# airframesio/aero-cli

Measured on AMD Instinct MI355X. Metric: Msamples/s demod+Viterbi, 10500bps OQPSK, 1/2/4/8 GPU; ACARS frames bit-exact vs ref, higher is better.
Workload: dtype f64

## Files before the change

### aero-cli_amd/aero_engine.py

```python
import ctypes
import os

import numpy as np

HERE = os.path.dirname(os.path.abspath(__file__))
LIB_PATH = os.path.join(HERE, 'libaero_engine.so')

AERO_OK = 0
AERO_E_INVALID = -1
AERO_E_NOMEM = -2
AERO_E_HIP = -3
AERO_E_NOGPU = -4
AERO_E_FULL = -5
AERO_E_RATE = -6
AERO_E_DEVICE = -7

F_TRACE_PT = 0x1
F_TRACE_BLOCKS = 0x2
F_TIMING = 0x4
F_TRACE_SOFT = 0x8
F_TRACE_HOPS = 0x10
F_TRACE_FRAMES = 0x20
F_DCD_TICK = 0x40
F_DCD_TICK_BURST = 0x80
F_DCD_TICK_CONT = 0x100
F_TRACE_ALL = F_TRACE_PT | F_TRACE_BLOCKS | F_TRACE_SOFT | F_TRACE_HOPS | F_TRACE_FRAMES

MATH_FN = {'hypot': 0, 'atan2': 1, 'tanh': 2, 'sin': 3, 'cos': 4, 'log10': 5, 'sqrt': 6, 'fmod360': 7,
           'div': 8, 'div_c48000': 9, 'div_c360': 10, 'div_n': 11, 'div_c192000': 13, 'hypot_nr': 14, 'atan2_bf': 15,
           'tanh_bf': 16, 'sin_bf': 17, 'cos_bf': 18,
           'div_cw_wt': 19, 'set_phase_ptr': 20, 'log10_ge1': 21}
VIT_VARIANT = {'wave': 0, 'regs': 1, 'regs2-self': 2, 'regs2-pair': 3, 'block4992': 4, 'block384': 5, 'block576': 6,
               'csoft': 7}
FFT_KIND = {'dit': 0, 'chain': 1}
VIT_BLOCK = {'block4992': 4992, 'block384': 384, 'block576': 576, 'csoft': 5460}


class EngineCfg(ctypes.Structure):
    _fields_ = [('device', ctypes.c_int), ('max_channels', ctypes.c_int), ('flags', ctypes.c_int)]


class ChannelCfg(ctypes.Structure):
    _fields_ = [('bitrate', ctypes.c_int), ('burst', ctypes.c_int), ('fs', ctypes.c_uint32),
                ('disable_reassembly', ctypes.c_int)]


class AcarsItem(ctypes.Structure):
    _fields_ = [('aesid', ctypes.c_uint32),
                ('gesid', ctypes.c_uint8), ('qno', ctypes.c_uint8), ('refno', ctypes.c_uint8),
                ('seqno', ctypes.c_uint8),
                ('mode', ctypes.c_uint8), ('tak', ctypes.c_uint8), ('bi', ctypes.c_uint8),
                ('nonacars', ctypes.c_uint8),
                ('downlink', ctypes.c_uint8), ('valid', ctypes.c_uint8), ('hastext', ctypes.c_uint8),
                ('moretocome', ctypes.c_uint8),
                ('fragment', ctypes.c_uint8), ('label_len', ctypes.c_uint8), ('reg_len', ctypes.c_uint8),
                ('pad0', ctypes.c_uint8),
                ('label', ctypes.c_char * 4), ('reg', ctypes.c_char * 16),
                ('msg_len', ctypes.c_uint32), ('msg', ctypes.c_char * 3584)]


class ChanCfg(ctypes.Structure):
    _fields_ = [('device', ctypes.c_int), ('sample_rate', ctypes.c_int), ('center_frequency', ctypes.c_int),
                ('mix_offset', ctypes.c_int), ('correct_dc_bias', ctypes.c_int), ('max_blocks', ctypes.c_int),
                ('flags', ctypes.c_int)]


class ChanMain(ctypes.Structure):
    _fields_ = [('frequency', ctypes.c_int), ('out_rate', ctypes.c_int), ('compress_scale', ctypes.c_int),
                ('publish', ctypes.c_int)]


class ChanVfo(ctypes.Structure):
    _fields_ = [('frequency', ctypes.c_int), ('data_rate', ctypes.c_int), ('out_rate', ctypes.c_int),
                ('filter_bandwidth', ctypes.c_int), ('gain', ctypes.c_float), ('skip', ctypes.c_int)]


CHAN_F_HOST_OUT = 0x1


class ChannelEvents(ctypes.Structure):
    _fields_ = [('dcd_edges', ctypes.c_int64), ('hunter_steps', ctypes.c_int64), ('hunter_fc', ctypes.c_double * 8)]


_SIGS = {
    'aero_engine_create': (ctypes.c_int, [ctypes.POINTER(EngineCfg), ctypes.POINTER(ctypes.c_void_p)]),
    'aero_engine_destroy': (None, [ctypes.c_void_p]),
    'aero_channel_open': (ctypes.c_int, [ctypes.c_void_p, ctypes.POINTER(ChannelCfg), ctypes.POINTER(ctypes.c_int)]),
    'aero_channel_close': (ctypes.c_int, [ctypes.c_void_p, ctypes.c_int]),
    'aero_engine_reserve': (ctypes.c_int, [ctypes.c_void_p, ctypes.POINTER(ChannelCfg), ctypes.c_int]),
    'aero_channel_export': (ctypes.c_int, [ctypes.c_void_p, ctypes.POINTER(ctypes.c_int), ctypes.c_int,
                                           ctypes.c_void_p, ctypes.c_size_t, ctypes.POINTER(ctypes.c_size_t)]),
    'aero_channel_import': (ctypes.c_int, [ctypes.c_void_p, ctypes.c_void_p, ctypes.c_size_t,
                                           ctypes.POINTER(ctypes.c_int), ctypes.c_int,
                                           ctypes.POINTER(ctypes.c_int)]),
    'aero_push_pcm': (ctypes.c_int, [ctypes.c_void_p, ctypes.c_int, ctypes.c_void_p, ctypes.c_size_t,
                                     ctypes.c_uint32]),
    'aero_push_pcm_batch': (ctypes.c_int, [ctypes.c_void_p, ctypes.c_void_p, ctypes.c_size_t, ctypes.c_size_t,
                                           ctypes.c_int, ctypes.c_int]),
    'aero_push_pcm_dev': (ctypes.c_int, [ctypes.c_void_p, ctypes.c_int, ctypes.c_void_p, ctypes.c_size_t,
                                         ctypes.c_uint32]),
    'aero_run': (ctypes.c_int, [ctypes.c_void_p]),
    'aero_flush': (ctypes.c_int, [ctypes.c_void_p]),
    'aero_pop_softbits': (ctypes.c_int, [ctypes.c_void_p, ctypes.c_int, ctypes.c_void_p, ctypes.c_size_t,
                                         ctypes.POINTER(ctypes.c_size_t)]),
    'aero_pop_items': (ctypes.c_int, [ctypes.c_void_p, ctypes.c_int, ctypes.POINTER(AcarsItem), ctypes.c_size_t,
                                      ctypes.POINTER(ctypes.c_size_t)]),
    'aero_pop_items_all': (ctypes.c_int, [ctypes.c_void_p, ctypes.POINTER(AcarsItem), ctypes.POINTER(ctypes.c_int),
                                          ctypes.c_size_t, ctypes.POINTER(ctypes.c_size_t)]),
    'aero_pop_hops': (ctypes.c_int, [ctypes.c_void_p, ctypes.c_int, ctypes.c_void_p, ctypes.c_size_t,
                                     ctypes.POINTER(ctypes.c_size_t)]),
    'aero_trace_select': (ctypes.c_int, [ctypes.c_void_p, ctypes.POINTER(ctypes.c_int), ctypes.c_int]),
    'aero_pop_pt': (ctypes.c_int, [ctypes.c_void_p, ctypes.c_int, ctypes.c_void_p, ctypes.c_size_t,
                                   ctypes.POINTER(ctypes.c_size_t)]),
    'aero_pop_blocks': (ctypes.c_int, [ctypes.c_void_p, ctypes.c_int, ctypes.c_void_p, ctypes.c_size_t,
                                       ctypes.POINTER(ctypes.c_size_t)]),
    'aero_pop_frames': (ctypes.c_int, [ctypes.c_void_p, ctypes.c_int, ctypes.c_void_p, ctypes.c_size_t,
                                       ctypes.POINTER(ctypes.c_size_t)]),
    'aero_pop_rt_tests': (ctypes.c_int, [ctypes.c_void_p, ctypes.c_int, ctypes.c_void_p, ctypes.c_size_t,
                                         ctypes.POINTER(ctypes.c_size_t)]),
    'aero_pop_c_units': (ctypes.c_int, [ctypes.c_void_p, ctypes.c_int, ctypes.c_void_p, ctypes.c_size_t,
                                        ctypes.POINTER(ctypes.c_size_t)]),
    'aero_pop_voice': (ctypes.c_int, [ctypes.c_void_p, ctypes.c_int, ctypes.c_void_p, ctypes.c_size_t,
                                      ctypes.POINTER(ctypes.c_size_t)]),
    'aero_pop_rt_packets': (ctypes.c_int, [ctypes.c_void_p, ctypes.c_int, ctypes.c_void_p, ctypes.c_size_t,
                                           ctypes.POINTER(ctypes.c_size_t)]),
    'aero_timing': (ctypes.c_int, [ctypes.c_void_p, ctypes.c_char_p, ctypes.POINTER(ctypes.c_double),
                                   ctypes.POINTER(ctypes.c_long)]),
    'aero_timing_reset': (None, [ctypes.c_void_p]),
    'aero_samples_processed': (ctypes.c_uint64, [ctypes.c_void_p]),
    'aero_stat': (ctypes.c_int, [ctypes.c_void_p, ctypes.c_char_p, ctypes.POINTER(ctypes.c_uint64)]),
    'aero_channel_stat': (ctypes.c_int, [ctypes.c_void_p, ctypes.c_int, ctypes.c_char_p,
                                         ctypes.POINTER(ctypes.c_int64)]),
    'aero_channel_get_events': (ctypes.c_int, [ctypes.c_void_p, ctypes.c_int, ctypes.POINTER(ChannelEvents)]),
    'aero_sync': (ctypes.c_int, [ctypes.c_void_p]),
    'aero_device_math': (ctypes.c_int, [ctypes.c_void_p, ctypes.c_int, ctypes.c_void_p, ctypes.c_void_p,
                                        ctypes.c_void_p, ctypes.c_size_t]),
    'aero_device_viterbi': (ctypes.c_int, [ctypes.c_void_p, ctypes.c_int, ctypes.c_void_p, ctypes.c_size_t,
                                           ctypes.c_size_t, ctypes.c_void_p, ctypes.c_void_p]),
    'aero_device_fft': (ctypes.c_int, [ctypes.c_void_p] + [ctypes.c_int] * 6 + [ctypes.c_void_p, ctypes.c_size_t,
                                                                                 ctypes.c_void_p]),
    'aero_channel_coarse_y': (ctypes.c_int, [ctypes.c_void_p, ctypes.c_int, ctypes.c_void_p, ctypes.c_size_t,
                                             ctypes.POINTER(ctypes.c_size_t), ctypes.POINTER(ctypes.c_int)]),
    'aero_strerror': (ctypes.c_char_p, [ctypes.c_int]),
    'aero_chan_create': (ctypes.c_int, [ctypes.POINTER(ChanCfg), ctypes.POINTER(ChanMain), ctypes.c_int,
                                        ctypes.POINTER(ChanVfo), ctypes.c_int, ctypes.POINTER(ctypes.c_void_p)]),
    'aero_chan_destroy': (None, [ctypes.c_void_p]),
    'aero_chan_block_len': (ctypes.c_int, [ctypes.c_void_p, ctypes.POINTER(ctypes.c_int)]),
    'aero_chan_vfo_info': (ctypes.c_int, [ctypes.c_void_p, ctypes.c_int, ctypes.POINTER(ctypes.c_int)]),
    'aero_chan_main_info': (ctypes.c_int, [ctypes.c_void_p, ctypes.c_int, ctypes.POINTER(ctypes.c_int)]),
    'aero_chan_push': (ctypes.c_int, [ctypes.c_void_p, ctypes.c_void_p, ctypes.c_size_t, ctypes.c_int]),
    'aero_chan_run': (ctypes.c_int, [ctypes.c_void_p]),
    'aero_chan_sync': (ctypes.c_int, [ctypes.c_void_p]),
    'aero_chan_vfo_output': (ctypes.c_int, [ctypes.c_void_p, ctypes.c_int, ctypes.POINTER(ctypes.c_void_p),
                                            ctypes.POINTER(ctypes.c_size_t)]),
    'aero_chan_pop_audio': (ctypes.c_int, [ctypes.c_void_p, ctypes.c_int, ctypes.c_void_p, ctypes.c_size_t,
                                           ctypes.POINTER(ctypes.c_size_t)]),
    'aero_chan_pop_iq': (ctypes.c_int, [ctypes.c_void_p, ctypes.c_int, ctypes.c_void_p, ctypes.c_size_t,
                                        ctypes.POINTER(ctypes.c_size_t)]),
    'aero_chan_feed': (ctypes.c_int, [ctypes.c_void_p, ctypes.c_void_p, ctypes.POINTER(ctypes.c_int)]),
    'aero_chan_vfo_open': (ctypes.c_int, [ctypes.c_void_p, ctypes.POINTER(ChanVfo), ctypes.POINTER(ctypes.c_int)]),
    'aero_chan_vfo_close': (ctypes.c_int, [ctypes.c_void_p, ctypes.c_int]),
    'aero_chan_vfo_skip': (ctypes.c_int, [ctypes.c_void_p, ctypes.c_int, ctypes.c_int]),
    'aero_chan_reserve': (ctypes.c_int, [ctypes.c_void_p, ctypes.POINTER(ChanVfo), ctypes.c_int]),
    'aero_chan_vfo_count': (ctypes.c_int, [ctypes.c_void_p, ctypes.POINTER(ctypes.c_int)]),
    'aero_chan_vfo_settle': (ctypes.c_int, [ctypes.c_void_p, ctypes.c_int, ctypes.POINTER(ctypes.c_size_t)]),
    'aero_chan_stat': (ctypes.c_int, [ctypes.c_void_p, ctypes.c_char_p, ctypes.POINTER(ctypes.c_uint64)]),
}

_lib = None


def _torch_hip_runtime():
    import importlib.util
    spec = importlib.util.find_spec('torch')
    if spec is None or not spec.origin:
        return []
    tlib = os.path.join(os.path.dirname(spec.origin), 'lib')
    return [p for p in (os.path.join(tlib, 'libhsa-runtime64.so'), os.path.join(tlib, 'libamdhip64.so'))
            if os.path.exists(p)]


def load_library(path=None):
    global _lib
    if _lib is not None:
        return _lib
    path = path or os.environ.get('AERO_ENGINE_SO') or LIB_PATH
    if not os.path.exists(path):
        raise RuntimeError('libaero_engine.so not built (%s); run aero-cli_amd/build.py' % path)
    for rt in _torch_hip_runtime():
        ctypes.CDLL(rt, mode=ctypes.RTLD_GLOBAL)
    lib = ctypes.CDLL(path)
    for name, (res, args) in _SIGS.items():
        try:
# ... 247 lines not shown
        self.lib.aero_timing_reset(self.h)

    def stat(self, name):
        v = ctypes.c_uint64()
        _check(self.lib.aero_stat(self.h, name.encode(), ctypes.byref(v)), 'aero_stat')
        return int(v.value)

    def channel_stat(self, ch, name):
        v = ctypes.c_int64()
        _check(self.lib.aero_channel_stat(self.h, ch, name.encode(), ctypes.byref(v)), 'aero_channel_stat')
        return int(v.value)

    def channel_events(self, ch):
        ev = ChannelEvents()
        _check(self.lib.aero_channel_get_events(self.h, ch, ctypes.byref(ev)), 'aero_channel_get_events')
        n = int(ev.hunter_steps)
        fcs = [ev.hunter_fc[(k - 1) & 7] for k in range(max(1, n - 7), n + 1)]
        return int(ev.dcd_edges), n, fcs

    def samples_processed(self):
        return int(self.lib.aero_samples_processed(self.h))

    def device_math(self, fn, x, y=None):
        x = np.ascontiguousarray(x, dtype=np.float64)
        y = np.zeros_like(x) if y is None else np.ascontiguousarray(y, dtype=np.float64)
        out = np.empty_like(x)
        _check(self.lib.aero_device_math(self.h, MATH_FN[fn], x.ctypes.data, y.ctypes.data, out.ctypes.data,
                                         x.size), 'aero_device_math')
        return out

    def device_viterbi(self, variant, rows, nsoft=None):
        rows = np.ascontiguousarray(rows, dtype=np.uint8)
        assert rows.ndim == 2
        src = variant in VIT_BLOCK
        nsoft = rows.shape[1] if nsoft is None else int(nsoft)
        bits = np.zeros((rows.shape[0], nsoft // 2), dtype=np.uint8)
        ov = np.zeros((rows.shape[0], 62), dtype=np.uint8)
        _check(self.lib.aero_device_viterbi(self.h, VIT_VARIANT[variant], rows.ctypes.data, rows.shape[0], nsoft,
                                            bits.ctypes.data, ov.ctypes.data if src else None),
               'aero_device_viterbi')
        return (bits, ov) if src else bits

    def device_fft(self, kind, records, inverse=False, depth=0, start=1, stop=0):
        records = np.ascontiguousarray(records, dtype=np.complex128)
        assert records.ndim == 2
        n = records.shape[1]
        log2n = n.bit_length() - 1 if n > 0 and n & (n - 1) == 0 else 0
        out = np.empty_like(records)
        _check(self.lib.aero_device_fft(self.h, FFT_KIND.get(kind, -1), log2n, int(inverse), int(depth), int(start),
                                        int(stop), records.ctypes.data, records.shape[0], out.ctypes.data),
               'aero_device_fft')
        return out

    def channel_coarse_y(self, ch):
        y = np.empty(16384, dtype=np.float64)
        n, first = ctypes.c_size_t(), ctypes.c_int()
        _check(self.lib.aero_channel_coarse_y(self.h, ch, y.ctypes.data, y.size, ctypes.byref(n), ctypes.byref(first)),
               'aero_channel_coarse_y')
        return int(first.value), y[:n.value].copy()


def vfo_out_rate(data_rate, out_rate=0):
    if out_rate or not data_rate:
        return out_rate
    return {600: 12000, 1200: 24000}.get(int(data_rate), 48000)


def vfo_bitrate(data_rate):
    return int(data_rate) if int(data_rate) in (600, 1200) else 10500


def parse_sdr_ini(text):
    sections, cur = {}, 'General'
    for raw in text.splitlines():
        line = raw.strip()
        if not line or line[0] in ';#':
            continue
        if line.startswith('[') and line.endswith(']'):
            cur = line[1:-1]
            continue
        if '=' in line:
            k, v = line.split('=', 1)
            sections.setdefault(cur, {})[k.strip()] = v.strip()

    def to_int(v):
        try:
            return int(v)
        except (TypeError, ValueError):
            return 0

    def to_float(v):
        try:
            return float(v)
        except (TypeError, ValueError):
            return 0.0

    def array(name):
        sec = sections.get(name, {})
        out = []
        for i in range(1, to_int(sec.get('size')) + 1):
            pre = '%d\\' % i
            out.append({k[len(pre):]: v for k, v in sec.items() if k.startswith(pre)})
        return out

    g = sections.get('General', {})
    general = dict(sample_rate=to_int(g.get('sample_rate')), center_frequency=to_int(g.get('center_frequency')),
# ... 142 lines not shown
```

### aero-cli_amd/build.py

```python
import argparse
import concurrent.futures as cf
import os
import shutil
import subprocess
import sys

HERE = os.path.dirname(os.path.abspath(__file__))
ROOT = os.path.dirname(HERE)
CSRC = os.path.join(HERE, 'csrc')
BUILD = os.path.join(HERE, 'build')
ENGINE_SO = os.path.join(HERE, 'libaero_engine.so')
SYNTH_SO = os.path.join(ROOT, 'tools', 'libaero_synth.so')
ORACLE_DIR = os.path.join(ROOT, 'oracle')

ARCH = os.environ.get('AERO_OFFLOAD_ARCH', 'gfx950')
HIPCC = os.environ.get('HIPCC', shutil.which('hipcc') or '/opt/rocm/bin/hipcc')
FP = ['-ffp-contract=off', '-fno-fast-math']
HIP_FLAGS = ['-O3', '-std=c++17', '-fPIC', '--offload-arch=' + ARCH] + FP
CXX_FLAGS = ['-O2', '-std=c++17', '-fPIC', '-Wall'] + FP

HIP_SRCS = ['demod_oqpsk.hip', 'demod_msk.hip', 'coarse.hip', 'aerol.hip', 'engine.hip', 'chan.hip', 'burst.hip', 'burst_msk.hip',
            'burst_engine.hip', 'cchan.hip', 'slot_reset.hip', 'slot_copy.hip', 'viterbi_probe.hip',
            'fft_probe.hip']
CXX_SRCS = ['tables_host.cpp', 'acars_host.cpp', 'chan_blob.cpp']
FILE_FLAGS = {'burst.hip': ['-mllvm', '-disable-machine-licm'],
              'burst_msk.hip': ['-mllvm', '-disable-machine-licm'],
              'demod_oqpsk.hip': ['-mllvm', '--amdgpu-sched-strategy=max-memory-clause', '-mllvm',
                                  '-disable-machine-licm'],
              'cchan.hip': ['-mllvm', '-disable-machine-licm'],
              'coarse.hip': ['-mllvm', '-disable-machine-licm']}


def _run(cmd):
    r = subprocess.run(cmd, capture_output=True, text=True)
    if r.returncode != 0:
        raise RuntimeError('build failed: %s\n%s%s' % (' '.join(cmd), r.stdout, r.stderr))
    return r


def _stale(out, deps):
    if not os.path.exists(out):
        return True
    t = os.path.getmtime(out)
    return any(os.path.getmtime(d) > t for d in deps)


def build_engine(jobs=4, variant=None, defines=(), file_flags=None):
    ff = dict(FILE_FLAGS, **(file_flags or {}))
    bdir = BUILD if variant is None else os.path.join(BUILD, variant)
    out = ENGINE_SO if variant is None else os.path.join(HERE, 'libaero_engine_%s.so' % variant)
    os.makedirs(bdir, exist_ok=True)
    headers = [os.path.join(CSRC, h) for h in os.listdir(CSRC) if h.endswith('.h')]
    headers += [os.path.join(ROOT, 'include', h) for h in ('aero_engine.h', 'aero_chan.h')]
    dflags = ['-D' + d for d in defines]
    tasks, objs = [], []
    for s in HIP_SRCS + CXX_SRCS:
        src = os.path.join(CSRC, s)
        obj = os.path.join(bdir, s + '.o')
        objs.append(obj)
        if _stale(obj, [src] + headers):
            if s.endswith('.hip'):
                cmd = [HIPCC] + HIP_FLAGS + ff.get(s, []) + dflags + ['-c', src, '-o', obj]
            else:
                cmd = ['g++'] + CXX_FLAGS + dflags + ['-c', src, '-o', obj]
            tasks.append(cmd)
    with cf.ThreadPoolExecutor(max_workers=max(1, jobs)) as ex:
        for f in [ex.submit(_run, t) for t in tasks]:
            f.result()
    if tasks or _stale(out, objs):
        _run([HIPCC, '--offload-arch=' + ARCH, '-shared', '-fPIC', '-o', out] + objs)
    return out


def build_synth():
    src = os.path.join(ROOT, 'tools', 'aero_synth.cpp')
    if _stale(SYNTH_SO, [src]):
        _run(['g++', '-O2', '-std=c++17', '-fPIC', '-shared', '-o', SYNTH_SO, src, '-lm'])
    return SYNTH_SO


MATHHOST_SO = os.path.join(ROOT, 'tools', 'libaero_mathhost.so')
FFTSIM_SO = os.path.join(ROOT, 'tools', 'libfft_chain_sim.so')


def build_fftsim():
    src = os.path.join(ROOT, 'tools', 'fft_chain_sim.cpp')
    if _stale(FFTSIM_SO, [src, os.path.join(CSRC, 'fft_layout.h')]):
        _run(['g++', '-O2', '-std=c++17', '-fPIC', '-shared', '-ffp-contract=off', '-o', FFTSIM_SO, src])
    return FFTSIM_SO


SCHEDSIM_SO = os.path.join(ROOT, 'tools', 'libcoarse_sched_sim.so')


def build_schedsim():
    src = os.path.join(ROOT, 'tools', 'coarse_sched_sim.cpp')
    if _stale(SCHEDSIM_SO, [src, os.path.join(CSRC, 'coarse_sched.h')]):
        _run(['g++', '-O2', '-std=c++17', '-Wall', '-fPIC', '-shared', '-o', SCHEDSIM_SO, src])
    return SCHEDSIM_SO


LDSSIM_SO = os.path.join(ROOT, 'tools', 'libcoarse_lds_sim.so')


def build_ldssim():
    src = os.path.join(ROOT, 'tools', 'coarse_lds_sim.cpp')
    if _stale(LDSSIM_SO, [src, os.path.join(CSRC, 'coarse_lds.h')]):
        _run(['g++', '-O2', '-std=c++17', '-Wall', '-fPIC', '-shared', '-o', LDSSIM_SO, src])
    return LDSSIM_SO


CHANSLOTS_SO = os.path.join(ROOT, 'tools', 'libchan_slots_sim.so')


def build_chanslots():
    src = os.path.join(ROOT, 'tools', 'chan_slots_sim.cpp')
    if _stale(CHANSLOTS_SO, [src, os.path.join(CSRC, 'chan_slots.h')]):
        _run(['g++', '-O2', '-std=c++17', '-Wall', '-fPIC', '-shared', '-o', CHANSLOTS_SO, src])
    return CHANSLOTS_SO


def build_mathhost():
    src = os.path.join(ROOT, 'tools', 'mathhost.cpp')
    deps = [src, os.path.join(CSRC, 'aero_math.h'), os.path.join(CSRC, 'aero_glibc_tables.h')]
    if _stale(MATHHOST_SO, deps):
        _run(['g++', '-O2', '-std=c++17', '-fPIC', '-shared', '-ffp-contract=off', '-o', MATHHOST_SO, src, '-lm'])
    return MATHHOST_SO


HOSTCHECK_SO = os.path.join(ROOT, 'tools', 'libaero_hostcheck.so')
HOSTCHECK_SRCS = [os.path.join(ROOT, 'tools', 'hostcheck.cpp'), os.path.join(CSRC, 'acars_host.cpp'),
                  os.path.join(CSRC, 'chan_blob.cpp'), os.path.join(CSRC, 'tables_host.cpp')]


def build_hostcheck(out=HOSTCHECK_SO, extra=()):
    deps = HOSTCHECK_SRCS + [os.path.join(CSRC, h) for h in ('acars_host.h', 'chan_blob.h', 'dcd_host.h', 'tables_host.h')]
    if _stale(out, deps):
        _run(['g++'] + CXX_FLAGS + list(extra) + ['-shared', '-o', out] + HOSTCHECK_SRCS + ['-lm'])
    return out


HOSTFUZZ = os.path.join(ROOT, 'tools', 'hostfuzz')


def build_hostfuzz(out=HOSTFUZZ):
    srcs = [os.path.join(ROOT, 'tools', 'hostfuzz_main.cpp'), os.path.join(CSRC, 'acars_host.cpp'),
            os.path.join(CSRC, 'chan_blob.cpp')]
    if _stale(out, srcs + [os.path.join(CSRC, h) for h in ('acars_host.h', 'chan_blob.h')]):
        _run(['g++', '-O1', '-g', '-std=c++17', '-Wall', '-fsanitize=address,undefined',
              '-fno-sanitize-recover=undefined', '-fno-omit-frame-pointer'] + FP + ['-o', out] + srcs)
    return out


def build_oracle():
    _run(['make', '-s', '-C', ORACLE_DIR])
    if os.path.isdir('/root/reference'):
        _run(['make', '-s', '-C', ORACLE_DIR, 'ref'])
    return os.path.join(ORACLE_DIR, 'liboracle.so')


ORACLETICK_SO = os.path.join(ROOT, 'tools', 'liboracle_tick.so')

# ... 170 lines not shown
```

### aero-cli_amd/csrc/coarse.hip

```cpp
#include <hip/hip_runtime.h>

#include <type_traits>

#include "aero_math.h"
#include "coarse_lds.h"
#include "coarse_sched.h"
#include "engine_common.h"
#include "fft_chain.h"

namespace aero {

#ifdef AERO_X_OCML
#define CO_HYPOT ::hypot
#define CO_HYPOT_NR ::hypot
#define CO_LOG10_GE1(x) ::log10(x)
#define CO_LOG10_GE1_TAB(x, tab) ::log10(x)
#else
#define CO_HYPOT aero_hypot
#define CO_HYPOT_NR aero_hypot_nr
#define CO_LOG10_GE1(x) aero_log10_ge1_w(x, &aero_g_log_tab[0][0])
#define CO_LOG10_GE1_TAB(x, tab) aero_log10_ge1_w(x, tab)
#endif

template <int M>
struct CoarseK;
template <>
struct CoarseK<MODE_OQPSK> {
  static constexpr int LOG2N = 14, HOPN = 4096, START = 3584, STOP = 12800, ILO = 4608, IHI = 11776, EPB = 1792;
  static constexpr int YLO = clds::YLO14, YHI = clds::YHI14;
  static constexpr double FS = 48000.0;
};
template <>
struct CoarseK<MODE_C8400> {
  static constexpr int LOG2N = 14, HOPN = 4096, START = 3584, STOP = 12800, ILO = 4608, IHI = 11776, EPB = 1434;
  static constexpr int YLO = clds::YLO14, YHI = clds::YHI14;
  static constexpr double FS = 48000.0;
};
template <int FS>
struct MskCoarseBins;
template <>
struct MskCoarseBins<12000> {
  static constexpr int START = 614, STOP = 7578, ILO = 3482, IHI = 4710, EPB = 205;
};
template <>
struct MskCoarseBins<24000> {
  static constexpr int START = 307, STOP = 7885, ILO = 3789, IHI = 4403, EPB = 102;
};
template <>
struct MskCoarseBins<48000> {
  static constexpr int START = 154, STOP = 8038, ILO = 3942, IHI = 4250, EPB = 51;
};
template <int M>
struct CoarseK {
  using B = MskCoarseBins<msk_fs(M)>;
  static constexpr int LOG2N = 13, HOPN = 2048, START = B::START, STOP = B::STOP, ILO = B::ILO, IHI = B::IHI,
                       EPB = B::EPB;
  static constexpr int YLO = MSK_YLO, YHI = MSK_YHI;
// ... 484 lines not shown
#pragma unroll
            for (int i = i0; i < i0 + 4; ++i) {
              x[i] = T.cis[0];
              pcmw[i >> 1] = 0;
            }
          }
        }
      };
      if constexpr (OVL) {
        static_assert((YLEN + FT - 1) / FT <= 12, "four groups of three iterations cover the bins");
        twv = make_double2(0.0, 0.0);
        constexpr int NIT = (YLEN + FT - 1) / FT;
        auto ystep = [&](double &yp, auto jc) {
          constexpr int j = decltype(jc)::value;
          constexpr bool full = (j + 1) * FT <= YLEN;
          static_assert(full || j >= NIT - 1, "one partial iteration, the last");
          if constexpr (j < NIT) {
            const int k = t + j * FT;
            if (full || uni(k) < YLEN) {
              const bool in = full || k < YLEN;
#ifdef AERO_X_NOYREAD
              double a = 20.0 * 0.9;
#else
              double a = ((in && !yreset) ? yp : 20.0) * 0.9;
              asm volatile("" : "+v"(a));
              if constexpr (j + 3 < NIT) yp = yg[min(k + 3 * FT, YLEN - 1)];
#endif
              const double lg = CO_LOG10_GE1_TAB(fmax(ylds[ypad(in ? k : YLEN - 1)], 1.0), sm.logtab);
              const double ynew = a + 0.1 * 10 * lg;
              if (in) ylds[ypad(k)] = ynew;
            }
          }
        };
        auto ygroup = [&](auto i0c) {
          constexpr int g = decltype(i0c)::value / 4;
          if (g == 3) twv = T.tw[min(t, TwLds<L>::LEN - 1)];
          gather4(i0c);
          ystep(yp0, std::integral_constant<int, 3 * g>());
          ystep(yp1, std::integral_constant<int, 3 * g + 1>());
          ystep(yp2, std::integral_constant<int, 3 * g + 2>());
        };
        ygroup(std::integral_constant<int, 0>());
        ygroup(std::integral_constant<int, 4>());
        ygroup(std::integral_constant<int, 8>());
        ygroup(std::integral_constant<int, 12>());
      } else {
#pragma unroll 1
        for (int k = t; k < YLEN; k += FT) ybody(k);
      }
      __syncthreads();
      CSTAMP(7);
      if constexpr (OVL) {
        if (nxt && t < TwLds<L>::LEN) s_tw[t] = twv;
#pragma unroll 1
        for (int k = t; k < YLEN; k += FT) yg[k] = ylds[ypad(k)];
        if (t < 64) ep = load_epi(S, C, c);
      }
      double bv = 0.0;
      int bi = 0x7fffffff;
      for (int r = 0;; ++r) {
        const int i = KB.ilo + t + FT * r;
        if (i >= KB.ihi) break;
        double val = 0;
        for (int j = -1; j <= 1; j++)
          val += (ylds[ypad(i - KB.epb - j - K::YLO)] + ylds[ypad(i + KB.epb + j - K::YLO)]);
        if (val > bv) {
          bv = val;
          bi = i;
        }
      }
      for (int off = 32; off > 0; off >>= 1) {
        const double ov = __shfl_down(bv, off, 64);
        const int oi = __shfl_down(bi, off, 64);
        if (ov > bv || (ov == bv && oi < bi)) {
          bv = ov;
          bi = oi;
        }
      }
      if ((t & 63) == 0) {
        red_v[t >> 6] = bv;
        red_i[t >> 6] = bi;
      }
      if (have_pro) pro = uni(pn);
      __syncthreads();
      CSTAMP(8);
      pre = OVL && nxt;
      if constexpr (OVL) {
        if (nxt) {
#pragma unroll
          for (int i = 0; i < 16; ++i) asm volatile("" : "+v"(x[i].x), "+v"(x[i].y));
#pragma unroll
          for (int i = 0; i < 16; ++i) {
            const uint32_t pw = pcmw[i >> 1];
            const double dv = ((double)(int16_t)((i & 1) ? (pw >> 16) : (pw & 0xFFFFu))) / 32768.0;
            x[i] = make_double2(x[i].x * dv, x[i].y * dv);
          }
          if (s0n < pn.zero_before) {
#pragma unroll
            for (int i = 0; i < 16; ++i) {
              const long long s = s0n + bitrev<L>(epos<L, 0>(t, i));
              if (s < pn.zero_before) x[i] = make_double2(0.0, 0.0);
            }
          }
        }
        CSTAMP(2);
      }
      if (t == 0) {
        if constexpr (!PERSIST) ep = load_epi(S, C, c);
        for (int w = 1; w < FT / 64; ++w) {
          if (red_v[w] > bv || (red_v[w] == bv && red_i[w] < bi)) {
            bv = red_v[w];
            bi = red_i[w];
          }
        }
        const int zmaxloc = (bv > 0.0) ? bi : N / 2;
        const double nfft = (double)N;
        const double freq_offset_est = -((double)(zmaxloc - nfft / 2)) * (KB.fs / nfft) * 0.5;
        double est;
        int ecd = ep.ecd;
        if (ecd <= 0) {
          est = freq_offset_est;
        } else {
          ecd--;
          est = 0;
        }

        double *ds = S.ds;
        int *is = S.is;
        const double mse = ep.mse;
        HopCtl h;
        h.m2f = ep.m2f;
        h.m2s = ep.m2s;
        h.mcf = ep.mcf;
        h.mcs = ep.mcs;
        h.countdown2 = ep.countdown2;
        h.countdown = ep.countdown;
        h.ecd = ecd;
        h.yres_next = 0;
        h.zb = zero_before;
        h.stepped = false;
        h.step_fc = 0.0;
        unsigned iter = (unsigned)ep.iter;
        int scans = ep.scans;
        const bool gotasignal = hop_control(h, std::integral_constant<int, M>(), KB.fs, est, mse, iter, scans, nk);
        is[IS_HUNT_ITER * C + c] = (int)iter;
        is[IS_HUNT_SCANS * C + c] = scans;
        if (h.stepped) {
          const int k = ep.steps;
          ds[(DS_HUNT_FC0 + (k & 7)) * C + c] = h.step_fc;
          is[IS_HUNT_STEPS * C + c] = k + 1;
        }
        ds[DS_M2_FREQ * C + c] = h.m2f;
        ds[DS_M2_STEP * C + c] = h.m2s;
        ds[DS_MC_FREQ * C + c] = h.mcf;
        ds[DS_MC_STEP * C + c] = h.mcs;
        is[IS_COUNTDOWN2 * C + c] = h.countdown2;
        is[IS_COUNTDOWN * C + c] = h.countdown;
        is[IS_EMPTYCD * C + c] = h.ecd;
        is[IS_YRESET * C + c] = h.yres_next;
        is[IS_HOPS_DONE * C + c] = hops_done + 1;
        S.ls[LS_ZERO_BEFORE * C + c] = h.zb;
        const int hn = ep.hop_n;
        if (hn < S.hop_cap) {
          double *hr = S.hops + ((size_t)c * S.hop_cap + hn) * 6;
          hr[0] = (double)nk;
          hr[1] = est;
          hr[2] = h.m2f;
          hr[3] = h.mcf;
// ... 68 lines not shown
```

### aero-cli_amd/csrc/engine.hip

```cpp
#include <hip/hip_runtime.h>

#include <algorithm>
#include <cmath>
#include <complex>
#include <cstdio>
#include <cstdlib>
#include <cstring>
#include <atomic>
#include <chrono>
#include <climits>
#include <deque>
#include <condition_variable>
#include <functional>
#include <mutex>
#include <new>
#include <map>
#include <memory>
#include <string>
#include <set>
#include <thread>
#include <type_traits>
#include <vector>

#include "../../include/aero_engine.h"
#include "acars_host.h"
#include "burst_engine.h"
#include "aero_math.h"
#include "chan_blob.h"
#include "dcd_host.h"
#include "engine_common.h"
#include "fft_layout.h"
#include "host_pool.h"
#include "engine_internal.h"
#include "slot_copy.h"
#include "slot_reset.h"
#include "tables_host.h"
#include "fft_probe.h"
#include "viterbi_probe.h"

namespace aero {
void launch_demod(hipStream_t, const DevState &, const DevTables &, int, int, bool, bool);
void upload_demod_constants(const double *, const DelayDesc *, const double *, const double *, const double *,
                            const double *);
void launch_demod_msk(hipStream_t, int, const DevState &, const DevTables &, int, int, bool);
void upload_msk_constants(const double *);
void demod_read_stamps(unsigned long long *);
void coarse_read_stamps(unsigned long long *);
void viterbi_read_stamps(unsigned long long *);
void burst_read_stamps(unsigned long long *);
void launch_coarse(hipStream_t, int, const DevState &, const DevTables &, int, int, bool);
void launch_frame(hipStream_t, int, const DevState &, int);
void launch_viterbi(hipStream_t, int, const DevState &, const DevTables &, int, int);
void launch_prefilter_c(hipStream_t, const DevState &, const DevTables &, const void *, int);
void launch_demod_c(hipStream_t, const DevState &, const DevTables &, int, bool);
void upload_c_constants(const DelayDesc *);
int c_prejob_bytes();
void launch_reset_slots(hipStream_t, void *, const ResetSeg *, int, const int *, const int *, int, const ResetInit *,
                        unsigned long long);
}

using namespace aero;

namespace {

constexpr int GENERIC_GROUP_CAP = 256;
constexpr long long PCM_CAP = 65536;
constexpr int PT_CAP = 4096;
constexpr int HOP_CAP = 64;

#define HIPCHK(x)                                   \
  do {                                              \
    hipError_t err__ = (x);                         \
    if (err__ != hipSuccess) {                      \
      fprintf(stderr, "aero_engine: %s failed: %s\n", #x, hipGetErrorString(err__)); \
      return AERO_E_HIP;                            \
    }                                               \
  } while (0)

__global__ void pcm_scatter_kernel(int16_t *ring, int C, long long capm, const int16_t *src, long long n, long long ld,
                                   int nch, int c0, long long start) {
  const long long total = n * nch;
  for (long long k = blockIdx.x * (long long)blockDim.x + threadIdx.x; k < total;
       k += (long long)gridDim.x * blockDim.x) {
    const long long t = k / nch;
    const int j = (int)(k - t * nch);
    ring[((start + t) & capm) * C + c0 + j] = src[t * ld + j];
  }
}

// ... 2540 lines not shown
    rec = (size_t)blk + 64;
    for (size_t k = 0; k < ncw; k++)
      if (in[k * rec + blk + 62] != (nsoft == (size_t)blk + 24 ? 1 : 0)) return AERO_E_INVALID;
  }
  HIPCHK(hipSetDevice(e->device));
  hipStream_t st = nullptr;
  const size_t nin = ncw * rec, nbits = ncw * (nsoft / 2), nov = ncw * 62;
  uint8_t *d = nullptr;
  HIPCHK(hipMalloc(&d, nin + nbits + nov + 64));
  HIPCHK(hipMemcpy(d, in, nin, hipMemcpyHostToDevice));
  launch_viterbi_probe(st, variant, d, (int)ncw, (int)nsoft, d + nin, d + nin + nbits);
  HIPCHK(hipGetLastError());
  HIPCHK(hipStreamSynchronize(st));
  HIPCHK(hipMemcpy(bits, d + nin, nbits, hipMemcpyDeviceToHost));
  if (blk) HIPCHK(hipMemcpy(overlap, d + nin + nbits, nov, hipMemcpyDeviceToHost));
  HIPCHK(hipFree(d));
  return AERO_OK;
}

int aero_device_fft(aero_engine *e, int kind, int log2n, int inverse, int depth, int start, int stop,
                    const double *in, size_t nrec, double *out) {
  if (!e || !in || !out || nrec < 1 || nrec > (size_t)FP_MAX_REC) return AERO_E_INVALID;
  if (!fft_probe_known(kind, log2n, inverse, depth)) return AERO_E_INVALID;
  const size_t nfft = (size_t)1 << log2n;
  std::vector<double> tw(2 * nfft), twi(2 * nfft), pg(2 * nfft, 0.0), pgi(2 * nfft, 0.0);
  host_twiddles((int)nfft, tw.data(), twi.data());
  if (kind == AERO_FFT_CHAIN) {
    if (log2n == 14) {
      fftl::twg_build<14>(tw.data(), pg.data());
      fftl::twg_build<14>(twi.data(), pgi.data());
    } else {
      fftl::twg_build<13>(tw.data(), pg.data());
      fftl::twg_build<13>(twi.data(), pgi.data());
    }
  }
  HIPCHK(hipSetDevice(e->device));
  hipStream_t st = nullptr;
  const size_t tb = sizeof(double) * 2 * nfft, rb = nrec * tb;
  char *d = nullptr;
  HIPCHK(hipMalloc(&d, 4 * tb + 2 * rb));
  const std::vector<double> *tabs[4] = {&tw, &twi, &pg, &pgi};
  for (int k = 0; k < 4; k++) HIPCHK(hipMemcpy(d + k * tb, tabs[k]->data(), tb, hipMemcpyHostToDevice));
  HIPCHK(hipMemcpy(d + 4 * tb, in, rb, hipMemcpyHostToDevice));
  auto tab = [&](int k) { return reinterpret_cast<const double2 *>(d + k * tb); };
  launch_fft_probe(st, kind, log2n, inverse, depth, start, stop, reinterpret_cast<const double2 *>(d + 4 * tb),
                   (int)nrec, reinterpret_cast<double2 *>(d + 4 * tb + rb), tab(0), tab(1), tab(2), tab(3));
  HIPCHK(hipGetLastError());
  HIPCHK(hipStreamSynchronize(st));
  HIPCHK(hipMemcpy(out, d + 4 * tb + rb, rb, hipMemcpyDeviceToHost));
  HIPCHK(hipFree(d));
  return AERO_OK;
}

int aero_channel_coarse_y(aero_engine *e, int ch, double *dst, size_t cap, size_t *n, int *first_bin) {
  if (!e || !dst || !n || !first_bin) return AERO_E_INVALID;
  if (route_burst(e, ch) >= 0) return AERO_E_INVALID;
  int c;
  Group *g = route(e, ch, c);
  if (!g) return AERO_E_INVALID;
  const size_t ylen = (size_t)(g->g.y_hi - g->g.y_lo + 1);
  if (cap < ylen) return AERO_E_INVALID;
  HIPCHK(hipSetDevice(e->device));
  if (int rc = flush_pending_init(g)) return rc;
  int yreset = 0;
  HIPCHK(hipMemcpyAsync(g->pin_stat, g->S.is + (size_t)IS_YRESET * g->C + c, sizeof(int), hipMemcpyDeviceToHost,
                        g->st));
  HIPCHK(hipMemcpyAsync(dst, g->S.y + (size_t)c * ylen, ylen * sizeof(double), hipMemcpyDeviceToHost, g->st));
  HIPCHK(hipStreamSynchronize(g->st));
  memcpy(&yreset, g->pin_stat, sizeof yreset);
  if (yreset)
    for (size_t k = 0; k < ylen; k++) dst[k] = 20.0;
  *n = ylen;
  *first_bin = g->g.y_lo;
  return AERO_OK;
}

}

int aero_engine_feed_dev(aero_engine *e, int nitems, const int *ch, const int16_t *const *src, const size_t *n,
                         const size_t *msg, const uint32_t *fs, hipEvent_t ready, hipStream_t producer) {
  if (!e || nitems < 0 || (nitems && (!ch || !src || !n || !msg || !fs))) return AERO_E_INVALID;
  for (int i = 0; i < nitems; i++)
    if (ch[i] >= 0 && ch[i] < (int)e->chmap.size() && e->chmap[ch[i]].first < 0) return AERO_E_INVALID;
  HIPCHK(hipSetDevice(e->device));
  std::vector<std::vector<FeedItem>> per(e->groups.size());
  std::vector<uint8_t> queued(e->chmap.size(), 0);
  auto feed_queued = [&]() -> int {
    for (size_t m = 0; m < per.size(); m++)
      if (!per[m].empty()) {
        if (int rc = feed_group(e->groups[m].get(), per[m], ready, producer)) return rc;
        per[m].clear();
      }
    std::fill(queued.begin(), queued.end(), 0);
    return AERO_OK;
  };
  for (int i = 0; i < nitems; i++) {
    if (!n[i]) continue;
    BurstGroup *bg;
    const int b = route_burst(e, ch[i], &bg);
    if (b >= 0) {
      HIPCHK(hipEventSynchronize(ready));
      const size_t m = msg[i] ? msg[i] : n[i];
      for (size_t p = 0; p < n[i]; p += m)
        if (int rc = push_burst(e, bg, b, src[i] + p, std::min(m, n[i] - p), true)) return rc;
      continue;
    }
// ... 109 lines not shown
```

### include/aero_engine.h

```cpp
#ifndef AERO_ENGINE_H
#define AERO_ENGINE_H

#include <stddef.h>
#include <stdint.h>

#ifdef __cplusplus
extern "C" {
#endif

#define AERO_OK 0
#define AERO_E_INVALID (-1)
#define AERO_E_NOMEM (-2)
#define AERO_E_HIP (-3)
#define AERO_E_NOGPU (-4)
#define AERO_E_FULL (-5)
#define AERO_E_RATE (-6)
#define AERO_E_DEVICE (-7)

#define AERO_F_TRACE_PT 0x1
#define AERO_F_TRACE_BLOCKS 0x2
#define AERO_F_TIMING 0x4
#define AERO_F_TRACE_SOFT 0x8
#define AERO_F_TRACE_HOPS 0x10
#define AERO_F_TRACE_FRAMES 0x20
// ... 54 lines not shown
int aero_pop_softbits(aero_engine *e, int ch, int16_t *dst, size_t cap, size_t *n);

int aero_pop_items(aero_engine *e, int ch, aero_acars_item *dst, size_t cap, size_t *n);

int aero_pop_items_all(aero_engine *e, aero_acars_item *dst, int *ch, size_t cap, size_t *n);

int aero_pop_hops(aero_engine *e, int ch, double *dst, size_t cap_records, size_t *n);
int aero_trace_select(aero_engine *e, const int *ch, int n);
int aero_pop_pt(aero_engine *e, int ch, double *dst, size_t cap_records, size_t *n);
int aero_pop_blocks(aero_engine *e, int ch, uint8_t *dst, size_t cap, size_t *n);
int aero_pop_frames(aero_engine *e, int ch, uint8_t *dst, size_t cap, size_t *n);
int aero_pop_rt_tests(aero_engine *e, int ch, uint8_t *dst, size_t cap, size_t *n);

int aero_pop_c_units(aero_engine *e, int ch, uint8_t *dst, size_t cap, size_t *n);
int aero_pop_voice(aero_engine *e, int ch, uint8_t *dst, size_t cap, size_t *n);
int aero_pop_rt_packets(aero_engine *e, int ch, uint8_t *dst, size_t cap, size_t *n);

int aero_timing(aero_engine *e, const char *name, double *ms, long *launches);
void aero_timing_reset(aero_engine *e);

int aero_stat(aero_engine *e, const char *name, uint64_t *value);

int aero_channel_stat(aero_engine *e, int ch, const char *name, int64_t *value);

typedef struct {
  int64_t dcd_edges;
  int64_t hunter_steps;
  double hunter_fc[8];
} aero_channel_events;
int aero_channel_get_events(aero_engine *e, int ch, aero_channel_events *out);

uint64_t aero_samples_processed(aero_engine *e);

int aero_sync(aero_engine *e);

int aero_device_math(aero_engine *e, int fn, const double *x, const double *y, double *out, size_t n);

#define AERO_VIT_WAVE 0
#define AERO_VIT_REGS 1
#define AERO_VIT_REGS2_SELF 2
#define AERO_VIT_REGS2_PAIR 3
#define AERO_VIT_BLOCK4992 4
#define AERO_VIT_BLOCK384 5
#define AERO_VIT_BLOCK576 6
#define AERO_VIT_CSOFT 7
int aero_device_viterbi(aero_engine *e, int variant, const uint8_t *in, size_t ncw, size_t nsoft, uint8_t *bits,
                        uint8_t *overlap);

#define AERO_FFT_DIT 0
#define AERO_FFT_CHAIN 1
int aero_device_fft(aero_engine *e, int kind, int log2n, int inverse, int depth, int start, int stop,
                    const double *in, size_t nrec, double *out);

int aero_channel_coarse_y(aero_engine *e, int ch, double *dst, size_t cap, size_t *n, int *first_bin);

const char *aero_strerror(int rc);

#ifdef __cplusplus
}
#endif
#endif
```

Before: 9350.

## Rewrite coarse fold peak search with contiguous per-thread runs and DPP wave reduction

In the persistent coarse-frequency kernel, each thread now scans a contiguous run of candidate bins and reuses a sliding window of LDS values instead of reloading six bins per candidate. The per-wave argmax reduction uses DPP row-shift and broadcast operations in place of __shfl_down, and the y copy-out loop is unrolled so loads are batched before stores. A probe kernel and host entry point are added to test the fold search on its own, along with a CPU simulator build, so bit-exact tie-breaking can be checked. The main risk is a mismatch in tie-breaking order, which the code handles by keeping the lower index on equal values.

Result: no change. 9410, median of 4 (+0.6%).

```diff
diff --git a/aero-cli_amd/aero_engine.py b/aero-cli_amd/aero_engine.py
--- a/aero-cli_amd/aero_engine.py
+++ b/aero-cli_amd/aero_engine.py
@@ -33,6 +33,8 @@
 VIT_VARIANT = {'wave': 0, 'regs': 1, 'regs2-self': 2, 'regs2-pair': 3, 'block4992': 4, 'block384': 5, 'block576': 6,
                'csoft': 7}
 FFT_KIND = {'dit': 0, 'chain': 1}
+FOLD_GEOM = {'oqpsk': 0, 'c': 1}
+FOLD_YLEN = 13568 - 2815 + 1
 VIT_BLOCK = {'block4992': 4992, 'block384': 384, 'block576': 576, 'csoft': 5460}
 
 
@@ -139,6 +141,8 @@
                                            ctypes.c_size_t, ctypes.c_void_p, ctypes.c_void_p]),
     'aero_device_fft': (ctypes.c_int, [ctypes.c_void_p] + [ctypes.c_int] * 6 + [ctypes.c_void_p, ctypes.c_size_t,
                                                                                  ctypes.c_void_p]),
+    'aero_device_fold': (ctypes.c_int, [ctypes.c_void_p, ctypes.c_int, ctypes.c_void_p, ctypes.c_size_t,
+                                        ctypes.c_void_p, ctypes.c_void_p]),
     'aero_channel_coarse_y': (ctypes.c_int, [ctypes.c_void_p, ctypes.c_int, ctypes.c_void_p, ctypes.c_size_t,
                                              ctypes.POINTER(ctypes.c_size_t), ctypes.POINTER(ctypes.c_int)]),
     'aero_strerror': (ctypes.c_char_p, [ctypes.c_int]),
@@ -492,6 +496,17 @@
                'aero_device_fft')
         return out
 
+    def device_fold(self, geom, records):
+        records = np.ascontiguousarray(records, dtype=np.float64)
+        assert records.ndim == 2
+        loc = np.empty(records.shape[0], dtype=np.int32)
+        best = np.empty(records.shape[0], dtype=np.float64)
+        if records.shape[1] != FOLD_YLEN:
+            raise AeroError(AERO_E_INVALID, 'aero_device_fold')
+        _check(self.lib.aero_device_fold(self.h, FOLD_GEOM.get(geom, -1), records.ctypes.data, records.shape[0],
+                                         loc.ctypes.data, best.ctypes.data), 'aero_device_fold')
+        return loc, best
+
     def channel_coarse_y(self, ch):
         y = np.empty(16384, dtype=np.float64)
         n, first = ctypes.c_size_t(), ctypes.c_int()
diff --git a/aero-cli_amd/build.py b/aero-cli_amd/build.py
--- a/aero-cli_amd/build.py
+++ b/aero-cli_amd/build.py
@@ -21,7 +21,7 @@
 
 HIP_SRCS = ['demod_oqpsk.hip', 'demod_msk.hip', 'coarse.hip', 'aerol.hip', 'engine.hip', 'chan.hip', 'burst.hip', 'burst_msk.hip',
             'burst_engine.hip', 'cchan.hip', 'slot_reset.hip', 'slot_copy.hip', 'viterbi_probe.hip',
-            'fft_probe.hip']
+            'fft_probe.hip', 'coarse_fold_probe.hip']
 CXX_SRCS = ['tables_host.cpp', 'acars_host.cpp', 'chan_blob.cpp']
 FILE_FLAGS = {'burst.hip': ['-mllvm', '-disable-machine-licm'],
               'burst_msk.hip': ['-mllvm', '-disable-machine-licm'],
@@ -108,6 +108,17 @@
     if _stale(LDSSIM_SO, [src, os.path.join(CSRC, 'coarse_lds.h')]):
         _run(['g++', '-O2', '-std=c++17', '-Wall', '-fPIC', '-shared', '-o', LDSSIM_SO, src])
     return LDSSIM_SO
+
+
+FOLDSIM_SO = os.path.join(ROOT, 'tools', 'libcoarse_fold_sim.so')
+
+
+def build_foldsim():
+    src = os.path.join(ROOT, 'tools', 'coarse_fold_sim.cpp')
+    if _stale(FOLDSIM_SO, [src, os.path.join(CSRC, 'coarse_fold.h'), os.path.join(CSRC, 'coarse_lds.h')]):
+        _run(['g++', '-O2', '-std=c++17', '-Wall', '-fPIC', '-shared', '-ffp-contract=off', '-fno-fast-math', '-o',
+              FOLDSIM_SO, src])
+    return FOLDSIM_SO
 
 
 CHANSLOTS_SO = os.path.join(ROOT, 'tools', 'libchan_slots_sim.so')
diff --git a/aero-cli_amd/csrc/coarse.hip b/aero-cli_amd/csrc/coarse.hip
--- a/aero-cli_amd/csrc/coarse.hip
+++ b/aero-cli_amd/csrc/coarse.hip
@@ -3,6 +3,7 @@
 #include <type_traits>
 
 #include "aero_math.h"
+#include "coarse_fold.h"
 #include "coarse_lds.h"
 #include "coarse_sched.h"
 #include "engine_common.h"
@@ -593,34 +594,49 @@
       CSTAMP(7);
       if constexpr (OVL) {
         if (nxt && t < TwLds<L>::LEN) s_tw[t] = twv;
-#pragma unroll 1
-        for (int k = t; k < YLEN; k += FT) yg[k] = ylds[ypad(k)];
+        constexpr int NIT = (YLEN + FT - 1) / FT, HALF = (NIT + 1) / 2;
+#pragma unroll
+        for (int h = 0; h < NIT; h += HALF) {
+          double yv[HALF];
+#pragma unroll
+          for (int j = 0; j < HALF; ++j)
+            if (h + j < NIT) yv[j] = ylds[ypad(min(t + (h + j) * FT, YLEN - 1))];
+#pragma unroll
+          for (int j = 0; j < HALF; ++j)
+            if (h + j < NIT && t + (h + j) * FT < YLEN) yg[t + (h + j) * FT] = yv[j];
+        }
         if (t < 64) ep = load_epi(S, C, c);
       }
       double bv = 0.0;
       int bi = 0x7fffffff;
-      for (int r = 0;; ++r) {
-        const int i = KB.ilo + t + FT * r;
-        if (i >= KB.ihi) break;
-        double val = 0;
-        for (int j = -1; j <= 1; j++)
-          val += (ylds[ypad(i - KB.epb - j - K::YLO)] + ylds[ypad(i + KB.epb + j - K::YLO)]);
-        if (val > bv) {
-          bv = val;
-          bi = i;
-        }
-      }
-      for (int off = 32; off > 0; off >>= 1) {
-        const double ov = __shfl_down(bv, off, 64);
-        const int oi = __shfl_down(bi, off, 64);
-        if (ov > bv || (ov == bv && oi < bi)) {
-          bv = ov;
-          bi = oi;
-        }
-      }
-      if ((t & 63) == 0) {
-        red_v[t >> 6] = bv;
-        red_i[t >> 6] = bi;
+      if constexpr (PERSIST) {
+        using FG = cfold::Geom<K::ILO, K::IHI, K::EPB, K::YLO, K::YHI, FT>;
+        static_assert(FG::pad(777) == fftl::ypadn<6>(777), "coarse_fold.h reads ylds by coarse_lds.h's padding");
+        cfold::scan_to_red<FG>(ylds, t, red_v, red_i);
+      } else {
+        for (int r = 0;; ++r) {
+          const int i = KB.ilo + t + FT * r;
+          if (i >= KB.ihi) break;
+          double val = 0;
+          for (int j = -1; j <= 1; j++)
+            val += (ylds[ypad(i - KB.epb - j - K::YLO)] + ylds[ypad(i + KB.epb + j - K::YLO)]);
+          if (val > bv) {
+            bv = val;
+            bi = i;
+          }
+        }
+        for (int off = 32; off > 0; off >>= 1) {
+          const double ov = __shfl_down(bv, off, 64);
+          const int oi = __shfl_down(bi, off, 64);
+          if (ov > bv || (ov == bv && oi < bi)) {
+            bv = ov;
+            bi = oi;
+          }
+        }
+        if ((t & 63) == 0) {
+          red_v[t >> 6] = bv;
+          red_i[t >> 6] = bi;
+        }
       }
       if (have_pro) pro = uni(pn);
       __syncthreads();
@@ -648,13 +664,17 @@
       }
       if (t == 0) {
         if constexpr (!PERSIST) ep = load_epi(S, C, c);
-        for (int w = 1; w < FT / 64; ++w) {
-          if (red_v[w] > bv || (red_v[w] == bv && red_i[w] < bi)) {
-            bv = red_v[w];
-            bi = red_i[w];
-          }
-        }
-        const int zmaxloc = (bv > 0.0) ? bi : N / 2;
+        if constexpr (PERSIST) {
+          cfold::best_of_red<cfold::Geom<K::ILO, K::IHI, K::EPB, K::YLO, K::YHI, FT>>(red_v, red_i, bv, bi);
+        } else {
+          for (int w = 1; w < FT / 64; ++w) {
+            if (red_v[w] > bv || (red_v[w] == bv && red_i[w] < bi)) {
+              bv = red_v[w];
+              bi = red_i[w];
+            }
+          }
+        }
+        const int zmaxloc = cfold::zmaxloc(bv, bi, N);
         const double nfft = (double)N;
         const double freq_offset_est = -((double)(zmaxloc - nfft / 2)) * (KB.fs / nfft) * 0.5;
         double est;
diff --git a/aero-cli_amd/csrc/coarse_fold.h b/aero-cli_amd/csrc/coarse_fold.h
--- /dev/null
+++ b/aero-cli_amd/csrc/coarse_fold.h
@@ -0,0 +1,114 @@
+#pragma once
+
+#include "coarse_lds.h"
+
+namespace aero {
+namespace cfold {
+
+template <int ILO_, int IHI_, int EPB_, int YLO_, int YHI_, int FT_>
+struct Geom {
+  static constexpr int ILO = ILO_, IHI = IHI_, EPB = EPB_, YLO = YLO_, YHI = YHI_, FT = FT_;
+  static constexpr int RUN = (IHI - ILO + FT - 1) / FT;
+  static constexpr int NONE = 0x7fffffff;
+  static_assert(ILO - EPB - 1 >= YLO && IHI - 1 + EPB + 1 <= YHI, "fold search inside the kept y bins");
+  static constexpr int first(int t) { return ILO + RUN * t < IHI ? ILO + RUN * t : IHI; }
+  static constexpr int end(int t) { return ILO + RUN * (t + 1) < IHI ? ILO + RUN * (t + 1) : IHI; }
+  static constexpr int lo_bin(int t, int k) { return first(t) - EPB - 1 + k; }
+  static constexpr int hi_bin(int t, int k) { return first(t) + EPB - 1 + k; }
+  static constexpr int pad(int q) { return clds::ypad(q); }
+  static constexpr int slot(int bin) { return pad(bin - YLO); }
+};
+
+#if defined(__HIPCC__)
+__host__ __device__
+#endif
+inline double candidate(double a0, double a1, double a2, double b0, double b1, double b2) {
+  double val = 0;
+  val += (a2 + b0);
+  val += (a1 + b1);
+  val += (a0 + b2);
+  return val;
+}
+
+#if defined(__HIPCC__)
+
+template <class G>
+__device__ __forceinline__ void scan(const double *ylds, int t, double &bv, int &bi) {
+  bv = 0.0;
+  bi = G::NONE;
+  const int i0 = G::first(t);
+  if (G::RUN * G::FT != G::IHI - G::ILO && i0 >= G::IHI) return;
+  const int lo = i0 - G::EPB - 1 - G::YLO, hi = i0 + G::EPB - 1 - G::YLO;
+  double a0 = ylds[G::pad(lo)], a1 = ylds[G::pad(lo + 1)];
+  double b0 = ylds[G::pad(hi)], b1 = ylds[G::pad(hi + 1)];
+#pragma unroll
+  for (int r = 0; r < G::RUN; ++r) {
+    const int i = i0 + r;
+    if (G::RUN * G::FT != G::IHI - G::ILO && i >= G::IHI) break;
+    const double a2 = ylds[G::pad(lo + r + 2)], b2 = ylds[G::pad(hi + r + 2)];
+    const double val = candidate(a0, a1, a2, b0, b1, b2);
+    if (val > bv) {
+      bv = val;
+      bi = i;
+    }
+    a0 = a1;
+    a1 = a2;
+    b0 = b1;
+    b1 = b2;
+  }
+}
+
+template <int CTRL, int ROW_MASK>
+__device__ __forceinline__ void take_dpp(double &bv, int &bi) {
+  const int vlo = __double2loint(bv), vhi = __double2hiint(bv);
+  const int olo = __builtin_amdgcn_update_dpp(vlo, vlo, CTRL, ROW_MASK, 0xf, false);
+  const int ohi = __builtin_amdgcn_update_dpp(vhi, vhi, CTRL, ROW_MASK, 0xf, false);
+  const int oi = __builtin_amdgcn_update_dpp(bi, bi, CTRL, ROW_MASK, 0xf, false);
+  const double ov = __hiloint2double(ohi, olo);
+  if (ov > bv || (ov == bv && oi < bi)) {
+    bv = ov;
+    bi = oi;
+  }
+}
+constexpr int DPP_ROW_SHR = 0x110, DPP_ROW_BCAST15 = 0x142, DPP_ROW_BCAST31 = 0x143;
+
+__device__ __forceinline__ void reduce_row(double &bv, int &bi) {
+  take_dpp<DPP_ROW_SHR + 1, 0xf>(bv, bi);
+  take_dpp<DPP_ROW_SHR + 2, 0xf>(bv, bi);
+  take_dpp<DPP_ROW_SHR + 4, 0xf>(bv, bi);
+  take_dpp<DPP_ROW_SHR + 8, 0xf>(bv, bi);
+}
+__device__ __forceinline__ void reduce_wave(double &bv, int &bi) {
+  reduce_row(bv, bi);
+  take_dpp<DPP_ROW_BCAST15, 0xa>(bv, bi);
+  take_dpp<DPP_ROW_BCAST31, 0xc>(bv, bi);
+}
+
+template <class G>
+__device__ __forceinline__ void scan_to_red(const double *ylds, int t, double *red_v, int *red_i) {
+  double bv;
+  int bi;
+  scan<G>(ylds, t, bv, bi);
+  reduce_wave(bv, bi);
+  if ((t & 63) == 63) {
+    red_v[t >> 6] = bv;
+    red_i[t >> 6] = bi;
+  }
+}
+template <class G>
+__device__ __forceinline__ void best_of_red(const double *red_v, const int *red_i, double &bv, int &bi) {
+  bv = red_v[0];
+  bi = red_i[0];
+  for (int w = 1; w < G::FT / 64; ++w) {
+    if (red_v[w] > bv || (red_v[w] == bv && red_i[w] < bi)) {
+      bv = red_v[w];
+      bi = red_i[w];
+    }
+  }
+}
+__device__ __forceinline__ int zmaxloc(double bv, int bi, int nfft) { return (bv > 0.0) ? bi : nfft / 2; }
+
+#endif
+
+}
+}
diff --git a/aero-cli_amd/csrc/coarse_fold_probe.h b/aero-cli_amd/csrc/coarse_fold_probe.h
--- /dev/null
+++ b/aero-cli_amd/csrc/coarse_fold_probe.h
@@ -0,0 +1,12 @@
+#pragma once
+#include <hip/hip_runtime.h>
+
+namespace aero {
+
+constexpr int FOLD_PROBE_MAX_REC = 1024;
+constexpr int FOLD_PROBE_NFFT = 16384;
+constexpr int FOLD_PROBE_YLEN = 13568 - 2815 + 1;
+
+void launch_fold_probe(hipStream_t st, int geom, const double *y, int nrec, int *loc, double *best);
+
+}
diff --git a/aero-cli_amd/csrc/coarse_fold_probe.hip b/aero-cli_amd/csrc/coarse_fold_probe.hip
--- /dev/null
+++ b/aero-cli_amd/csrc/coarse_fold_probe.hip
@@ -0,0 +1,44 @@
+#include <hip/hip_runtime.h>
+
+#include "coarse_fold.h"
+#include "coarse_fold_probe.h"
+
+namespace aero {
+
+namespace {
+
+template <class G>
+__global__ __launch_bounds__(G::FT, 1) void fold_probe_kernel(const double *y, int *loc, double *best) {
+  constexpr int YLEN = G::YHI - G::YLO + 1, YSPAN = clds::ypad(YLEN - 1) + 1;
+  static_assert(YLEN == FOLD_PROBE_YLEN, "the record length the host copies");
+  __shared__ double ylds[YSPAN];
+  __shared__ double red_v[G::FT / 64];
+  __shared__ int red_i[G::FT / 64];
+  const int t = threadIdx.x;
+  const double *rec = y + (size_t)blockIdx.x * YLEN;
+  for (int k = t; k < YLEN; k += G::FT) ylds[clds::ypad(k)] = rec[k];
+  __syncthreads();
+  cfold::scan_to_red<G>(ylds, t, red_v, red_i);
+  __syncthreads();
+  if (t == 0) {
+    double bv;
+    int bi;
+    cfold::best_of_red<G>(red_v, red_i, bv, bi);
+    loc[blockIdx.x] = cfold::zmaxloc(bv, bi, FOLD_PROBE_NFFT);
+    best[blockIdx.x] = bv;
+  }
+}
+
+using FoldOqpsk = cfold::Geom<4608, 11776, 1792, clds::YLO14, clds::YHI14, 1024>;
+using FoldCchan = cfold::Geom<4608, 11776, 1434, clds::YLO14, clds::YHI14, 1024>;
+
+}
+
+void launch_fold_probe(hipStream_t st, int geom, const double *y, int nrec, int *loc, double *best) {
+  if (geom == 0)
+    hipLaunchKernelGGL(fold_probe_kernel<FoldOqpsk>, dim3(nrec), dim3(1024), 0, st, y, loc, best);
+  else
+    hipLaunchKernelGGL(fold_probe_kernel<FoldCchan>, dim3(nrec), dim3(1024), 0, st, y, loc, best);
+}
+
+}
diff --git a/aero-cli_amd/csrc/engine.hip b/aero-cli_amd/csrc/engine.hip
--- a/aero-cli_amd/csrc/engine.hip
+++ b/aero-cli_amd/csrc/engine.hip
@@ -35,6 +35,7 @@
 #include "slot_copy.h"
 #include "slot_reset.h"
 #include "tables_host.h"
+#include "coarse_fold_probe.h"
 #include "fft_probe.h"
 #include "viterbi_probe.h"
 
@@ -2681,6 +2682,25 @@
   return AERO_OK;
 }
 
+int aero_device_fold(aero_engine *e, int geom, const double *y, size_t nrec, int *zmaxloc, double *best) {
+  if (!e || !y || !zmaxloc || !best || nrec < 1 || nrec > (size_t)FOLD_PROBE_MAX_REC) return AERO_E_INVALID;
+  if (geom != AERO_FOLD_OQPSK && geom != AERO_FOLD_C) return AERO_E_INVALID;
+  HIPCHK(hipSetDevice(e->device));
+  hipStream_t st = nullptr;
+  const size_t yb = nrec * FOLD_PROBE_YLEN * sizeof(double), lb = (nrec * sizeof(int) + 7) / 8 * 8;
+  char *d = nullptr;
+  HIPCHK(hipMalloc(&d, yb + lb + nrec * sizeof(double)));
+  HIPCHK(hipMemcpy(d, y, yb, hipMemcpyHostToDevice));
+  launch_fold_probe(st, geom, reinterpret_cast<const double *>(d), (int)nrec, reinterpret_cast<int *>(d + yb),
+                    reinterpret_cast<double *>(d + yb + lb));
+  HIPCHK(hipGetLastError());
+  HIPCHK(hipStreamSynchronize(st));
+  HIPCHK(hipMemcpy(zmaxloc, d + yb, nrec * sizeof(int), hipMemcpyDeviceToHost));
+  HIPCHK(hipMemcpy(best, d + yb + lb, nrec * sizeof(double), hipMemcpyDeviceToHost));
+  HIPCHK(hipFree(d));
+  return AERO_OK;
+}
+
 int aero_channel_coarse_y(aero_engine *e, int ch, double *dst, size_t cap, size_t *n, int *first_bin) {
   if (!e || !dst || !n || !first_bin) return AERO_E_INVALID;
   if (route_burst(e, ch) >= 0) return AERO_E_INVALID;
diff --git a/include/aero_engine.h b/include/aero_engine.h
--- a/include/aero_engine.h
+++ b/include/aero_engine.h
@@ -130,6 +130,10 @@
 int aero_device_fft(aero_engine *e, int kind, int log2n, int inverse, int depth, int start, int stop,
                     const double *in, size_t nrec, double *out);
 
+#define AERO_FOLD_OQPSK 0
+#define AERO_FOLD_C 1
+int aero_device_fold(aero_engine *e, int geom, const double *y, size_t nrec, int *zmaxloc, double *best);
+
 int aero_channel_coarse_y(aero_engine *e, int ch, double *dst, size_t cap, size_t *n, int *first_bin);
 
 const char *aero_strerror(int rc);
```
